# RuihanGao/visual-tactile-synthesis

Hardware: AMD Instinct MI355X
Metric: train_images_per_sec (higher is better)
Workload: dtype f32; 1 GPU; skitG G+D1+D2 train step, 1024x1024 sketch->(RGB,tactile), 4 images/GPU, 64 tactile patches/image, LPIPS/CLIP terms off (no weights offline); global_batch=4, parallelism=dp1, losses_finite=True, hip_graph=True, d2_visualisation_pass=True, train_only=False, full=False

## Files before the change

### visual-tactile-synthesis_amd/csrc/vts_conv_head.hip

```cpp
#include <limits.h>
#include <stdlib.h>

#include "vts_internal.h"

namespace {

struct HeadK {
  const float* x;
  const float *sc, *sh;
  int64_t ns;
  int C, IH, IW, OH, OW, pad, padx;
  const float* w;
  int ws_ci;
  const float* bias;
  float* out;
  int64_t ons;
  float slope;
  const float* ident;
};

constexpr int HK_TY = 32, HK_TX = 32, HK_PR = HK_TY + 3, HK_PC = HK_TX + 3, HK_PCP = 36;
constexpr int HK_MAXC = 512;

template <int CK>
__global__ __launch_bounds__(1024) void conv_head_kernel(const HeadK p) {
  constexpr int BLOCK = 1024, NG = BLOCK / 256, CPG = CK / NG;
  static_assert(CK % NG == 0, "a chunk splits evenly over the thread groups");
  constexpr int NEL = CK * HK_PR * HK_PC;
  constexpr int NLD = (NEL + BLOCK - 1) / BLOCK;
  __shared__ __attribute__((aligned(16))) float tile[CK][HK_PR][HK_PCP];
  __shared__ __attribute__((aligned(16))) float wl[CK][16];
  __shared__ float ssc[HK_MAXC], ssh[HK_MAXC];
  const int tid = threadIdx.x, n = blockIdx.z;
  const int grp = __builtin_amdgcn_readfirstlane(tid >> 8), t256 = tid & 255;
  const int tx4 = t256 & 7, ty = t256 >> 3;
  const int oy0 = blockIdx.y * HK_TY, ox0 = blockIdx.x * HK_TX;
  const int iy0 = oy0 - p.pad, ix0 = ox0 - p.padx;
  for (int c = tid; c < p.C; c += BLOCK) {
    ssc[c] = p.sc ? p.sc[n * p.C + c] : 1.f;
    ssh[c] = p.sh ? p.sh[n * p.C + c] : 0.f;
  }
  int soff[NLD], sdst[NLD];
  const int64_t plane = (int64_t)p.IH * p.IW;
#pragma unroll
  for (int i = 0; i < NLD; ++i) {
    const int e = i * BLOCK + tid;
    const int c = e / (HK_PR * HK_PC), rem = e - c * (HK_PR * HK_PC);
    const int r = rem / HK_PC, col = rem - r * HK_PC;
    const int iy = iy0 + r, ix = ix0 + col;
    const bool in = e < NEL && iy >= 0 && iy < p.IH && ix >= 0 && ix < p.IW;
    soff[i] = in ? iy * p.IW + ix : -1;
    sdst[i] = e < NEL ? (c * HK_PR + r) * HK_PCP + col : -1;
  }
  const float* xb = p.x + n * p.ns;
  float pv[NLD];
  static_assert(BLOCK <= HK_PR * HK_PC, "one boundary per slot");
  auto chan = [&](int i) {
    const int b = (i * BLOCK) / (HK_PR * HK_PC);
    return b + (tid >= (b + 1) * (HK_PR * HK_PC) - i * BLOCK ? 1 : 0);
  };
  auto load_chunk = [&](int c0) {
#pragma unroll
    for (int i = 0; i < NLD; ++i) {
      const int c = c0 + chan(i);
      pv[i] = (soff[i] >= 0 && c < p.C) ? xb[c * plane + soff[i]] : 0.f;
    }
  };
  auto store_chunk = [&](int c0) {
    float* t = &tile[0][0][0];
#pragma unroll
    for (int i = 0; i < NLD; ++i) {
      const int c = c0 + chan(i);
      if (sdst[i] >= 0) {
        const bool ok = soff[i] >= 0 && c < p.C;
        const int cc = min(c, p.C - 1);
        const float u = fmaf(pv[i], ssc[cc], ssh[cc]);
        t[sdst[i]] = ok ? fmaxf(u, 0.f) + p.slope * fminf(u, 0.f) : 0.f;
      }
    }
    if (tid < CK * 16) {
      const int c = c0 + (tid >> 4);
      wl[tid >> 4][tid & 15] = c < p.C ? p.w[(int64_t)c * p.ws_ci + (tid & 15)] : 0.f;
    }
  };
  float acc[4] = {0.f, 0.f, 0.f, 0.f};
  __syncthreads();
  load_chunk(0);
  store_chunk(0);
  __syncthreads();
  for (int c0 = 0; c0 < p.C; c0 += CK) {
    const bool more = c0 + CK < p.C;
    if (more) load_chunk(c0 + CK);
#pragma unroll
    for (int cg = 0; cg < CPG; ++cg) {
      const int c = grp * CPG + cg;
#pragma unroll
      for (int ky = 0; ky < 4; ++ky) {
        const f32x4 a = *reinterpret_cast<const f32x4*>(&tile[c][ty + ky][tx4 * 4]);
        const f32x4 b = *reinterpret_cast<const f32x4*>(&tile[c][ty + ky][tx4 * 4 + 4]);
        const f32x4 wv = *reinterpret_cast<const f32x4*>(&wl[c][ky * 4]);
        const float v[8] = {a[0], a[1], a[2], a[3], b[0], b[1], b[2], b[3]};
#pragma unroll
        for (int kx = 0; kx < 4; ++kx)
#pragma unroll
          for (int j = 0; j < 4; ++j) acc[j] = fmaf(v[j + kx], wv[kx], acc[j]);
      }
    }
    __syncthreads();
    if (more) {
      store_chunk(c0 + CK);
      __syncthreads();
    }
  }
  f32x4* red = reinterpret_cast<f32x4*>(&tile[0][0][0]);
  if (grp > 0) red[(grp - 1) * 256 + t256] = (f32x4){acc[0], acc[1], acc[2], acc[3]};
  __syncthreads();
  if (grp > 0) return;
#pragma unroll
  for (int g = 1; g < NG; ++g) {
    const f32x4 v = red[(g - 1) * 256 + t256];
#pragma unroll
    for (int j = 0; j < 4; ++j) acc[j] += v[j];
  }
  const float bias = p.bias ? p.bias[0] : 0.f;
  const int y = oy0 + ty;
  if (y < p.OH) {
    float* o = p.out + n * p.ons + (int64_t)y * p.OW;
#pragma unroll
    for (int j = 0; j < 4; ++j) {
      const int x = ox0 + tx4 * 4 + j;
      if (x < p.OW) o[x] = acc[j] + bias;
    }
  }
}

struct HeadSK {
  const float* x;
  const float *sc, *sh;
  int64_t ns;
  int C, N, IH, IW, OH, OW, pad, padx;
  const float* w;
  int ws_ci;
  const float* bias;
  float* out;
  int64_t ons;
  float slope;
  int IPB, PH, PW, CK;
};

__global__ __launch_bounds__(256) void conv_head_small_kernel(const HeadSK p) {
  extern __shared__ __attribute__((aligned(16))) float smem[];
  float* tile = smem;
  float* wl = smem + p.IPB * p.CK * p.PH * p.PW;
  const int tid = threadIdx.x;
  const int n0 = blockIdx.x * p.IPB;
  const int nimg = min(p.IPB, p.N - n0);
  const int plane = p.PH * p.PW, ohw = p.OH * p.OW, ihw = p.IH * p.IW;
  const int img = tid / ohw, r = tid - img * ohw;
  const int oy = r / p.OW, ox = r - oy * p.OW;
  const bool active = img < nimg;
  const int base = img * p.CK * plane + oy * p.PW + ox;
  for (int i = tid; i < p.IPB * p.CK * plane; i += 256) tile[i] = 0.f;
  float acc = 0.f;
  for (int c0 = 0; c0 < p.C; c0 += p.CK) {
    __syncthreads();
    const int total = nimg * p.CK * ihw;
    for (int e0 = tid; e0 < total; e0 += 256 * 8) {
      float raw[8], fsc[8], fsh[8];
      int dst[8];
#pragma unroll
      for (int j = 0; j < 8; ++j) {
        const int e = e0 + j * 256;
        const int ee = min(e, total - 1);
        const int ic = ee / ihw, q = ee - ic * ihw;
        const int im = ic / p.CK, c = ic - im * p.CK;
        const int y = q / p.IW, x = q - y * p.IW;
        const int cc = min(c0 + c, p.C - 1), n = n0 + im;
        raw[j] = p.x[n * p.ns + (int64_t)cc * ihw + q];
        fsc[j] = p.sc ? p.sc[n * p.C + cc] : 1.f;
        fsh[j] = p.sh ? p.sh[n * p.C + cc] : 0.f;
        dst[j] = (e < total && c0 + c < p.C) ? (im * p.CK + c) * plane + (y + p.pad) * p.PW + x + p.padx : -1 - ((im * p.CK + c) * plane + (y + p.pad) * p.PW + x + p.padx);
        if (e >= total) dst[j] = INT_MIN;
      }
#pragma unroll
      for (int j = 0; j < 8; ++j) {
        const float t = fmaf(raw[j], fsc[j], fsh[j]);
        if (dst[j] >= 0) tile[dst[j]] = fmaxf(t, 0.f) + p.slope * fminf(t, 0.f);
        else if (dst[j] != INT_MIN) tile[-1 - dst[j]] = 0.f;
      }
    }
    for (int e = tid; e < p.CK * 16; e += 256) wl[e] = (c0 + (e >> 4) < p.C) ? p.w[(int64_t)(c0 + (e >> 4)) * p.ws_ci + (e & 15)] : 0.f;
    __syncthreads();
    if (active) {
#pragma unroll 4
      for (int c = 0; c < p.CK; ++c) {
        const float* t = tile + base + c * plane;
#pragma unroll
        for (int ky = 0; ky < 4; ++ky)
#pragma unroll
          for (int kx = 0; kx < 4; ++kx) acc = fmaf(t[ky * p.PW + kx], wl[c * 16 + ky * 4 + kx], acc);
      }
    }
  }
  if (active) p.out[(n0 + img) * p.ons + r] = acc + (p.bias ? p.bias[0] : 0.f);
}

}

int vts_conv_head_try(const vts_conv_desc* d, hipStream_t st) {
  static const int off = vts_tune_set("VTS_NO_HEAD") ? 1 : 0;
  if (off || d->transposed || d->stride != 1 || d->Cout != 1 || d->in1.data || d->dmask.data || d->accumulate || d->act_out != VTS_ACT_NONE)
    return VTS_ERR_UNSUPPORTED;
  if (d->in0.C > HK_MAXC || d->in0.C < 8 || (int64_t)d->IH * d->IW * d->in0.C >= (1ll << 31)) return VTS_ERR_UNSUPPORTED;
  if ((int64_t)d->OH * d->OW < 1024) {
    const int padx = d->pad + d->pad_dx;
    if (d->N < 32 || d->OH * d->OW > 256 || d->pad < 0 || padx < 0 || d->IH + d->pad < d->OH + 3 - d->pad || d->IW + padx < d->OW + 3 - padx)
      return VTS_ERR_UNSUPPORTED;
    HeadSK q;
    q.x = d->in0.data; q.sc = d->in0.scale; q.sh = d->in0.shift; q.ns = d->in0.nstride; q.C = d->in0.C; q.N = d->N;
    q.IH = d->IH; q.IW = d->IW; q.OH = d->OH; q.OW = d->OW; q.pad = d->pad; q.padx = padx;
    q.w = d->w; q.ws_ci = d->ws_ci; q.bias = d->bias; q.out = d->out; q.ons = d->out_nstride; q.slope = vts_slope(d->act_in);
    q.PH = d->IH + 2 * d->pad; q.PW = d->IW + 2 * padx;
    q.IPB = 256 / (d->OH * d->OW);
    q.CK = d->in0.C;
    auto bytes = [&]() { return (int64_t)(q.IPB * q.CK * q.PH * q.PW + q.CK * 16) * 4; };
    while (q.IPB > 2 && bytes() > 60 * 1024) --q.IPB;
    if (bytes() > 60 * 1024) {
      q.CK = 16;
      q.IPB = 256 / (d->OH * d->OW);
      while (q.IPB > 1 && bytes() > 60 * 1024) --q.IPB;
    }
    const int lds = (int)bytes();
    if (lds > 64 * 1024) return VTS_ERR_UNSUPPORTED;
    hipLaunchKernelGGL(conv_head_small_kernel, dim3(cdiv(d->N, q.IPB)), dim3(256), lds, st, q);
    vts_set_kernel("conv_head_small_kernel");
    VTS_CHECK_LAUNCH("vts_conv4x4 (head, small maps)");
    return VTS_OK;
  }
  HeadK k;
  k.x = d->in0.data; k.sc = d->in0.scale; k.sh = d->in0.shift; k.ns = d->in0.nstride; k.C = d->in0.C;
  k.IH = d->IH; k.IW = d->IW; k.OH = d->OH; k.OW = d->OW; k.pad = d->pad; k.padx = d->pad + d->pad_dx;
  k.w = d->w; k.ws_ci = d->ws_ci; k.bias = d->bias; k.out = d->out; k.ons = d->out_nstride;
  k.slope = vts_slope(d->act_in);
  k.ident = nullptr;
  dim3 grid(cdiv(d->OW, HK_TX), cdiv(d->OH, HK_TY), d->N);
  hipLaunchKernelGGL((conv_head_kernel<8>), grid, dim3(1024), 0, st, k);
  vts_set_kernel("conv_head_kernel<8>");
  VTS_CHECK_LAUNCH("vts_conv4x4 (head)");
  return VTS_OK;
}
```

### visual-tactile-synthesis_amd/csrc/vts_wgrad.hip

```cpp
#include <stdio.h>
#include <stdlib.h>

#include "vts_internal.h"

namespace {

struct Src {
  const float *d0, *d1, *sc0, *sh0, *sc1, *sh1;
  int64_t ns0, ns1;
  int C0, C1, C;
  int act;
  float slope;
  const float* ident;
  int plain;
};

struct WgK {
  Src lo, hi;
  int N, LH, LW, HH, HW, pad, padx;
  int cl_groups, ch_groups;
  int tiles_y, tiles_x, ntiles;
  float* part;
  int ablate;
};
// ... 520 lines not shown
        live[j] = img < nimg;
      }
#pragma unroll
      for (int j = 0; j < 8; ++j) {
        const float t = fmaf(raw[j], fsc[j], fsh[j]);
        if (dst[j] >= 0) lo_t[dst[j]] = live[j] ? fmaxf(t, 0.f) + p.lo_slope * fminf(t, 0.f) : 0.f;
      }
    }
    const int hi_total = nimg * p.CH * hhw;
    for (int e0 = tid; e0 < hi_total; e0 += 256 * 8) {
      float raw[8], fsc[8], fsh[8];
      int dst[8];
#pragma unroll
      for (int j = 0; j < 8; ++j) {
        const int e = min(e0 + j * 256, hi_total - 1);
        int r, c, x;
        const int ic = fdiv(e, hhw, inv_hhw, r);
        const int img = fdiv(ic, p.CH, inv_ch, c);
        const int y = fdiv(r, p.HW, inv_hw, x);
        const int n = n0 + img;
        raw[j] = p.hi[n * p.hins + (int64_t)c * hhw + r];
        fsc[j] = p.hisc ? p.hisc[n * p.CH + c] : 1.f;
        fsh[j] = p.hish ? p.hish[n * p.CH + c] : 0.f;
        dst[j] = e0 + j * 256 < hi_total ? img * imgstride + c * p.PLANE + (y + SW_HALO) * p.PW_ + x + SW_HALO : -1;
      }
#pragma unroll
      for (int j = 0; j < 8; ++j) {
        const float t = fmaf(raw[j], fsc[j], fsh[j]);
        if (dst[j] >= 0) hi_t[dst[j]] = fmaxf(t, 0.f) + p.hi_slope * fminf(t, 0.f);
      }
    }
    __syncthreads();
    const int ngroups = (nimg * lhw + 3) >> 2;
    constexpr int UG = (CLT * CHW >= 16) ? 2 : 4;
    for (int g0 = 0; g0 < ngroups; g0 += UG) {
      float a[UG][CLT], b[UG][CHW];
#pragma unroll
      for (int u = 0; u < UG; ++u) {
        const int pos = min(g0 + u, ngroups - 1) * 4 + kq;
#pragma unroll
        for (int t = 0; t < CLT; ++t) a[u][t] = lo_t[(t * 16 + m16) * p.POSP + pos];
        const int base = postab[pos] + tapoff;
#pragma unroll
        for (int c = 0; c < CHW; ++c) b[u][c] = hi_t[base + min(wave * CHW + c, p.CH - 1) * p.PLANE];
      }
#pragma unroll
      for (int u = 0; u < UG; ++u) {
        if (g0 + u < ngroups) {
#pragma unroll
          for (int t = 0; t < CLT; ++t)
#pragma unroll
            for (int c = 0; c < CHW; ++c) acc[t][c] = __builtin_amdgcn_mfma_f32_16x16x4f32(a[u][t], b[u][c], acc[t][c], 0, 0, 0);
        }
      }
    }
    __syncthreads();
  }
  float* part = p.part + (int64_t)blockIdx.x * p.CL * p.CH * 16;
#pragma unroll
  for (int t = 0; t < CLT; ++t)
#pragma unroll
    for (int c = 0; c < CHW; ++c) {
      const int ch = wave * CHW + c;
#pragma unroll
      for (int r = 0; r < 4; ++r) {
        const int cl = t * 16 + kq * 4 + r;
        if (cl < p.CL && ch < p.CH) part[((int64_t)cl * p.CH + ch) * 16 + m16] = acc[t][c][r];
      }
    }
}

struct HeadWK {
  const float* lo;
  int64_t lons;
  const float *hi, *hisc, *hish;
  int64_t hins;
  int CH, N, LH, LW, HH, HW, pad, padx;
  float hi_slope;
  int tiles_y, tiles_x;
  float* part;
};
constexpr int HWG_TY = 16, HWG_TX = 32, HWG_PR = HWG_TY + 3, HWG_PC = HWG_TX + 3, HWG_PCP = 36, HWG_CK = 16, HWG_PLANE = HWG_PR * HWG_PCP;

__global__ __launch_bounds__(256) void wgrad_head_kernel(const HeadWK p) {
  __shared__ __attribute__((aligned(16))) float patch[HWG_CK * HWG_PLANE];
  __shared__ __attribute__((aligned(16))) float dyt[HWG_TY * HWG_PCP];
  const int tid = threadIdx.x;
  const int tile = blockIdx.x;
  const int n = tile / (p.tiles_y * p.tiles_x), rem = tile - n * (p.tiles_y * p.tiles_x);
  const int ty = rem / p.tiles_x, tx = rem - ty * p.tiles_x;
  const int y0 = ty * HWG_TY, x0 = tx * HWG_TX;
  const int hy0 = y0 - p.pad, hx0 = x0 - p.padx;
  for (int e = tid; e < HWG_TY * HWG_TX; e += 256) {
    const int r = e >> 5, c = e & 31;
    const int y = y0 + r, x = x0 + c;
    dyt[r * HWG_PCP + c] = (y < p.LH && x < p.LW) ? p.lo[n * p.lons + (int64_t)y * p.LW + x] : 0.f;
  }
  const int rg = tid & 3, ky = (tid >> 2) & 3, chl = tid >> 4;
  const int64_t hplane = (int64_t)p.HH * p.HW;
  float* part = p.part + (int64_t)tile * p.CH * 16;
  const int lane = tid & 63;
  const int wv = __builtin_amdgcn_readfirstlane(tid >> 6);
  const int ix = hx0 + lane;
  const bool colok = lane < HWG_PC && ix >= 0 && ix < p.HW;
  const int ixc = min(max(ix, 0), p.HW - 1);
  float raw[HWG_CK / 4][HWG_PR];
  auto load_chunk = [&](int c0) {
#pragma unroll
    for (int cc = 0; cc < HWG_CK / 4; ++cc) {
      const int chc = min(c0 + wv + 4 * cc, p.CH - 1);
      const float* src = p.hi + n * p.hins + chc * hplane + ixc;
#pragma unroll
      for (int r = 0; r < HWG_PR; ++r) raw[cc][r] = src[(int64_t)min(max(hy0 + r, 0), p.HH - 1) * p.HW];
    }
  };
  auto store_chunk = [&](int c0) {
#pragma unroll
    for (int cc = 0; cc < HWG_CK / 4; ++cc) {
      const int c = wv + 4 * cc, ch = c0 + c;
      const bool chok = ch < p.CH;
      const int chc = chok ? ch : p.CH - 1;
      const float sc = p.hisc ? p.hisc[n * p.CH + chc] : 1.f, sh = p.hish ? p.hish[n * p.CH + chc] : 0.f;
      float* dstp = patch + c * HWG_PLANE + min(lane, HWG_PCP - 1);
#pragma unroll
      for (int r = 0; r < HWG_PR; ++r) {
        const int iy = hy0 + r;
        const bool ok = chok && colok && iy >= 0 && iy < p.HH;
        const float t = fmaf(raw[cc][r], sc, sh);
        if (lane < HWG_PCP) dstp[r * HWG_PCP] = ok ? fmaxf(t, 0.f) + p.hi_slope * fminf(t, 0.f) : 0.f;
      }
    }
  };
  load_chunk(0);
  for (int c0 = 0; c0 < p.CH; c0 += HWG_CK) {
    __syncthreads();
    store_chunk(c0);
    if (c0 + HWG_CK < p.CH) load_chunk(c0 + HWG_CK);
    __syncthreads();
    float acc[4] = {0.f, 0.f, 0.f, 0.f};
#pragma unroll
    for (int j = 0; j < HWG_TY / 4; ++j) {
      const int r = rg + 4 * j;
      const f32x4* vp = reinterpret_cast<const f32x4*>(patch + chl * HWG_PLANE + (r + ky) * HWG_PCP);
      const f32x4* dp = reinterpret_cast<const f32x4*>(dyt + r * HWG_PCP);
      float v[HWG_PCP], d[HWG_TX];
#pragma unroll
      for (int i = 0; i < HWG_PCP / 4; ++i) {
        const f32x4 t = vp[i];
        v[4 * i] = t[0]; v[4 * i + 1] = t[1]; v[4 * i + 2] = t[2]; v[4 * i + 3] = t[3];
      }
#pragma unroll
      for (int i = 0; i < HWG_TX / 4; ++i) {
        const f32x4 t = dp[i];
        d[4 * i] = t[0]; d[4 * i + 1] = t[1]; d[4 * i + 2] = t[2]; d[4 * i + 3] = t[3];
      }
#pragma unroll
      for (int x = 0; x < HWG_TX; ++x)
#pragma unroll
        for (int kx = 0; kx < 4; ++kx) acc[kx] = fmaf(d[x], v[x + kx], acc[kx]);
    }
#pragma unroll
    for (int kx = 0; kx < 4; ++kx) {
      const float a = acc[kx] + __shfl_xor(acc[kx], 1);
      acc[kx] = a + __shfl_xor(a, 2);
    }
    if (rg == 0 && c0 + chl < p.CH) *reinterpret_cast<f32x4*>(part + (c0 + chl) * 16 + ky * 4) = (f32x4){acc[0], acc[1], acc[2], acc[3]};
  }
}

__global__ __launch_bounds__(1024) void wgrad_reduce_kernel(const float* __restrict__ part, int64_t n, int pw, float* __restrict__ dw,
                                                            int accumulate) {
  __shared__ float red[16][64];
  const int lane = threadIdx.x & 63, w = threadIdx.x >> 6;
  const int64_t i = (int64_t)blockIdx.x * 64 + lane;
  float s = 0.f;
  if (i < n)
    for (int k = w; k < pw; k += 16) s += part[(int64_t)k * n + i];
  red[w][lane] = s;
  __syncthreads();
  if (w == 0 && i < n) {
    float t = 0.f;
#pragma unroll
    for (int k = 0; k < 16; ++k) t += red[k][lane];
    dw[i] = accumulate ? dw[i] + t : t;
  }
}

constexpr int RB_JOBS = 40;
struct ReduceTable {
  int njobs;
  int blk_start[RB_JOBS + 1];
  unsigned char narrow[RB_JOBS];
  vts_reduce_job job[RB_JOBS];
};

constexpr int RB_ELEMS = 256;
__global__ __launch_bounds__(1024) void wgrad_reduce_batch_kernel(const ReduceTable t) {
  __shared__ f32x4 red[16][64];
  int lo = 0, hi = t.njobs - 1;
  while (lo < hi) {
    const int mid = (lo + hi + 1) >> 1;
    if (t.blk_start[mid] <= (int)blockIdx.x) lo = mid;
    else hi = mid - 1;
  }
  const vts_reduce_job& j = t.job[lo];
  const int lane = threadIdx.x & 63, w = threadIdx.x >> 6;
  if (t.narrow[lo]) {
    const int el = lane & 15, cg = lane >> 4;
    const int64_t nb = (int64_t)(blockIdx.x - t.blk_start[lo]) * 64;
    f32x4 sn = {0.f, 0.f, 0.f, 0.f};
    for (int sg = 0; sg < j.nseg; ++sg) {
      const float* part = j.part[sg];
      const int pw = j.pw[sg];
      const bool vec = nb + 64 <= j.nel && (j.nel & 3) == 0 && (reinterpret_cast<uintptr_t>(part) & 15) == 0;
      f32x4 a[8];
#pragma unroll
      for (int u = 0; u < 8; ++u) a[u] = (f32x4){0.f, 0.f, 0.f, 0.f};
      for (int k = w * 4 + cg; k < pw; k += 512) {
#pragma unroll
        for (int u = 0; u < 8; ++u) {
// ... 268 lines not shown
bool dispatch_ns(const WgK& k, const Plan& pl, hipStream_t st) {
  if (S == 2 && pl.ty > 2) {
#define TALL_CASE(CLT, CHT, TY) \
  if (pl.clt == CLT && pl.cht == CHT && pl.ty == TY) { launch_ns_tall<CLT, CHT, TY>(k, pl, st); return true; }
    TALL_CASE(1, 1, 8) TALL_CASE(2, 1, 8)
#undef TALL_CASE
    return false;
  }
#define NS_CASE(CLT, CHT) \
  if (pl.clt == CLT && pl.cht == CHT) { launch_ns<S, CLT, CHT>(k, pl, st); return true; }
#define NS_ROW(CLT) NS_CASE(CLT, 1) NS_CASE(CLT, 2) NS_CASE(CLT, 3) NS_CASE(CLT, 4) NS_CASE(CLT, 5)
  NS_ROW(1) NS_ROW(2) NS_ROW(3) NS_ROW(4) NS_ROW(5)
#undef NS_ROW
#undef NS_CASE
  return false;
}

}


extern "C" int64_t vts_wgrad4x4_ws_floats(const vts_wgrad_desc* d) {
  if (!d) return 0;
  const int64_t CL = d->lo0.C + (d->lo1.data ? d->lo1.C : 0), CH = d->hi0.C + (d->hi1.data ? d->hi1.C : 0);
  const Plan pl = make_plan(d);
  return (int64_t)pl.pw * CL * CH * 16;
}

extern "C" int vts_wgrad4x4(const vts_wgrad_desc* d, float* ws, void* stream) {
  VTS_CHECK_ARG(d && d->lo0.data && d->hi0.data && d->dw && ws, "vts_wgrad4x4: null pointer");
  VTS_CHECK_ARG(d->stride == 1 || d->stride == 2, "vts_wgrad4x4: stride %d unsupported", d->stride);
  VTS_CHECK_ARG(d->LH <= d->HH + 16 && d->LW <= d->HW + 16 && d->pad >= -8 && d->pad <= 8,
                "vts_wgrad4x4: lo %dx%d / pad %d implausible for hi %dx%d s%d", d->LH, d->LW, d->pad, d->HH, d->HW, d->stride);
  const Plan pl = make_plan(d);
  WgK k;
  fill_src(k.lo, d->lo0, d->lo1, d->act_lo);
  fill_src(k.hi, d->hi0, d->hi1, d->act_hi);
  k.N = d->N; k.LH = d->LH; k.LW = d->LW; k.HH = d->HH; k.HW = d->HW; k.pad = d->pad; k.padx = d->pad + d->pad_dx;
  k.cl_groups = pl.cl_groups; k.ch_groups = pl.ch_groups;
  k.tiles_y = pl.tiles_y; k.tiles_x = pl.tiles_x; k.ntiles = pl.ntiles;
  k.part = ws;
  static const int ablate = vts_tune("VTS_ABLATE", 0);
  k.ablate = ablate;
  hipStream_t st = (hipStream_t)stream;
  const int64_t nel = (int64_t)k.lo.C * k.hi.C * 16;
  if (pl.small) {
    SmallWK q;
    q.lo = d->lo0.data; q.losc = d->lo0.scale; q.losh = d->lo0.shift; q.lons = d->lo0.nstride;
    q.hi = d->hi0.data; q.hisc = d->hi0.scale; q.hish = d->hi0.shift; q.hins = d->hi0.nstride;
    q.CL = k.lo.C; q.CH = k.hi.C; q.N = d->N; q.LH = d->LH; q.LW = d->LW; q.HH = d->HH; q.HW = d->HW; q.S = d->stride; q.pad = d->pad;
    q.padx = d->pad + d->pad_dx;
    q.lo_slope = vts_slope(d->act_lo); q.hi_slope = vts_slope(d->act_hi);
    q.IPB = pl.ipb; q.nblocks = pl.nblocks; q.POS = pl.pos; q.POSP = pl.posp; q.PW_ = pl.pwf; q.PLANE = pl.plane;
    q.part = ws;
    bool ok = false;
#define SW_CASE(CLT, CHW)                                                                                                      \
  if (pl.clt == CLT && pl.cht == CHW) {                                                                                        \
    static bool attr = false;                                                                                                  \
    if (!attr) {                                                                                                               \
      (void)hipFuncSetAttribute((const void*)wgrad_small_kernel<CLT, CHW>, hipFuncAttributeMaxDynamicSharedMemorySize, 160 * 1024); \
      attr = true;                                                                                                             \
    }                                                                                                                          \
    hipLaunchKernelGGL((wgrad_small_kernel<CLT, CHW>), dim3(pl.pw), dim3(256), pl.lds_bytes, st, q);                           \
    vts_set_kernel("wgrad_small_kernel<%d, %d>", CLT, CHW);                                                                    \
    ok = true;                                                                                                                 \
  }
    SW_CASE(1, 2) SW_CASE(1, 4) SW_CASE(1, 8) SW_CASE(1, 16) SW_CASE(2, 2) SW_CASE(2, 4) SW_CASE(2, 8) SW_CASE(2, 16) SW_CASE(4, 2) SW_CASE(4, 4)
    SW_CASE(4, 8)
#undef SW_CASE
    VTS_CHECK_ARG(ok, "vts_wgrad4x4: no small-map instance for clt %d chw %d", pl.clt, pl.cht);
    VTS_CHECK_LAUNCH("vts_wgrad4x4 (small maps)");
    if (d->defer) return VTS_OK;
    hipLaunchKernelGGL(wgrad_reduce_kernel, dim3((unsigned)cdiv64(nel, 64)), dim3(1024), 0, st, ws, nel, pl.pw, d->dw, d->accumulate);
    VTS_CHECK_LAUNCH("vts_wgrad4x4 reduce");
    return VTS_OK;
  }
  if (pl.head) {
    HeadWK q;
    q.lo = d->lo0.data; q.lons = d->lo0.nstride;
    q.hi = d->hi0.data; q.hisc = d->hi0.scale; q.hish = d->hi0.shift; q.hins = d->hi0.nstride;
    q.CH = k.hi.C; q.N = d->N; q.LH = d->LH; q.LW = d->LW; q.HH = d->HH; q.HW = d->HW; q.pad = d->pad; q.padx = d->pad + d->pad_dx;
    q.hi_slope = vts_slope(d->act_hi);
    q.tiles_y = pl.tiles_y; q.tiles_x = pl.tiles_x;
    q.part = ws;
    hipLaunchKernelGGL(wgrad_head_kernel, dim3(pl.ntiles), dim3(256), 0, st, q);
    vts_set_kernel("wgrad_head_kernel");
    VTS_CHECK_LAUNCH("vts_wgrad4x4 (single channel)");
    if (d->defer) return VTS_OK;
    hipLaunchKernelGGL(wgrad_reduce_kernel, dim3((unsigned)cdiv64(nel, 64)), dim3(1024), 0, st, ws, nel, pl.pw, d->dw, d->accumulate);
    VTS_CHECK_LAUNCH("vts_wgrad4x4 reduce");
    return VTS_OK;
  }
  if (pl.ns) {
    const bool ok = d->stride == 2 ? dispatch_ns<2>(k, pl, st) : dispatch_ns<1>(k, pl, st);
    VTS_CHECK_ARG(ok, "vts_wgrad4x4: no N-split instance for clt %d cht %d", pl.clt, pl.cht);
    VTS_CHECK_LAUNCH("vts_wgrad4x4 (N-split)");
    if (d->defer) return VTS_OK;
    hipLaunchKernelGGL(wgrad_reduce_kernel, dim3((unsigned)cdiv64(nel, 64)), dim3(1024), 0, st, ws, nel, pl.pw, d->dw, d->accumulate);
    VTS_CHECK_LAUNCH("vts_wgrad4x4 reduce");
    return VTS_OK;
  }
#define WG_CASE(S, CLT, CHT) \
  if (d->stride == S && pl.clt == CLT && pl.cht == CHT) launch_wg<S, CLT, CHT>(k, pl, st);
  WG_CASE(2, 1, 4) WG_CASE(2, 1, 10) WG_CASE(2, 2, 4) WG_CASE(2, 2, 10) WG_CASE(2, 3, 4) WG_CASE(2, 3, 10) WG_CASE(2, 5, 4)
  WG_CASE(1, 1, 4) WG_CASE(1, 1, 10) WG_CASE(1, 2, 4) WG_CASE(1, 2, 10) WG_CASE(1, 3, 4) WG_CASE(1, 3, 10) WG_CASE(1, 5, 4)
#undef WG_CASE
  VTS_CHECK_LAUNCH("vts_wgrad4x4");
  if (d->defer) return VTS_OK;
  hipLaunchKernelGGL(wgrad_reduce_kernel, dim3((unsigned)cdiv64(nel, 64)), dim3(1024), 0, st, ws, nel, pl.pw, d->dw,
                     d->accumulate);
  VTS_CHECK_LAUNCH("vts_wgrad4x4 reduce");
  return VTS_OK;
}

extern "C" int vts_wgrad_reduce_batch(const vts_reduce_job* jobs, int njobs, void* stream) {
  VTS_CHECK_ARG(jobs && njobs >= 0, "vts_wgrad_reduce_batch: null pointer");
  hipStream_t st = (hipStream_t)stream;
  for (int j0 = 0; j0 < njobs; j0 += RB_JOBS) {
    ReduceTable t;
    t.njobs = njobs - j0 < RB_JOBS ? njobs - j0 : RB_JOBS;
    int blocks = 0;
    for (int j = 0; j < t.njobs; ++j) {
      const vts_reduce_job& q = jobs[j0 + j];
      VTS_CHECK_ARG(q.dw && q.nel > 0 && q.nseg >= 1 && q.nseg <= VTS_REDUCE_MAX_SEG, "vts_wgrad_reduce_batch: bad job %d", j0 + j);
      for (int sg = 0; sg < q.nseg; ++sg) VTS_CHECK_ARG(q.part[sg] && q.pw[sg] >= 1, "vts_wgrad_reduce_batch: bad segment %d of job %d", sg, j0 + j);
      t.job[j] = q;
      t.blk_start[j] = blocks;
      int maxpw = 0;
      for (int sg = 0; sg < q.nseg; ++sg) maxpw = q.pw[sg] > maxpw ? q.pw[sg] : maxpw;
      static const int narrow_min = vts_tune("VTS_REDUCE_NARROW_MIN", 256);
      t.narrow[j] = maxpw > narrow_min ? 1 : 0;
      blocks += (int)cdiv64(q.nel, t.narrow[j] ? 64 : RB_ELEMS);
    }
    t.blk_start[t.njobs] = blocks;
    hipLaunchKernelGGL(wgrad_reduce_batch_kernel, dim3((unsigned)blocks), dim3(1024), 0, st, t);
    VTS_CHECK_LAUNCH("vts_wgrad_reduce_batch");
  }
  return VTS_OK;
}
```

### visual-tactile-synthesis_amd/vts/ops.py

```python
import ctypes as C
import os
from . import tune

import torch

from . import lib as L


class Act:

    __slots__ = ("data", "scale", "shift", "mean", "rstd", "padded")

    def __init__(self, data, scale=None, shift=None, mean=None, rstd=None):
        self.data, self.scale, self.shift, self.mean, self.rstd = data, scale, shift, mean, rstd
        self.padded = None

    @property
    def shape(self):
        return self.data.shape

    def operand(self):
        return L.operand(self.data, self.scale, self.shift)


TIMER = None


DETAIL = None


KNOCKOUT = tuple(k for k in tune.get("VTS_KNOCKOUT", "").split(",") if k)


def _run(label, nbytes, flops, fn, *args):
    global DETAIL
    if KNOCKOUT and label.startswith(KNOCKOUT):
        return
    if TIMER is None:
        L.check(fn(*args), label)
        return
    e0, e1 = torch.cuda.Event(enable_timing=True), torch.cuda.Event(enable_timing=True)
    e0.record()
    rc = fn(*args)
    e1.record()
    L.check(rc, label)
    if label.startswith(("conv4x4", "wgrad4x4", "patch_conv4x4", "patch_wgrad4x4", "norm_", "conv3x3_wide", "wgrad3x3_wide")):
        label = L.load().vts_last_kernel().decode()
    TIMER.append((label, nbytes, flops, e0, e1, DETAIL))
    DETAIL = None


def _numel(op):
    return 0


_ws = {}


def workspace(nfloats, device):
    key = (str(device), WS_LANE)
    t = _ws.get(key)
    if t is None or t.numel() < nfloats:
        if t is not None and frozen_ws():
            _retired.append(t)
        t = torch.empty(max(int(nfloats), 2 * (t.numel() if t is not None else 0), 1 << 20), dtype=torch.float32, device=device)
        _ws[key] = t
    return t


_retired = []

_counters = {}
FUSE_FINALIZE = tune.get("VTS_FUSE_FINALIZE", "0") == "1"


def counters(device):
    if not FUSE_FINALIZE:
        return None
    key = (str(device), WS_LANE)
    t = _counters.get(key)
    if t is None:
        t = _counters[key] = torch.zeros(1 << 16, dtype=torch.int32, device=device)
    return t


_WS_HOLDERS = set()


def freeze_ws(owner):
    _WS_HOLDERS.add(owner)


def release_ws(owner):
    _WS_HOLDERS.discard(owner)


def frozen_ws():
    return bool(_WS_HOLDERS)


WS_LANE = 0


def _op(a):
    if a is None:
        return L.Operand(None, None, None, 0, 0)
    if isinstance(a, Act):
        return a.operand()
    if isinstance(a, L.Operand):
        return a
    return L.operand(a)


BWD_SUMS = tune.get("VTS_BWD_SUMS", "1") != "0"
# ... 1319 lines not shown
```

Baseline: 762.0 images/s.

## Rework single-channel head conv and wgrad kernels for occupancy and register prefetch

The large-map head conv moves from a 1024-thread block with a 32x32 tile to a 256-thread, 8-row tile. Each wave now loads whole input columns into registers, double-buffered, and all weights are staged once in dynamic LDS. The small-map head kernel replaces integer division with magic-number multiplies, loads more elements per batch, and reads weights as vector loads. The head wgrad kernel gains a 512-thread variant that splits channels across two halves when there are fewer tiles than compute units, and it prefetches the per-channel affine terms alongside the data. These changes aim at better occupancy and latency hiding in the discriminator head passes, at the cost of more registers and LDS, and dynamic LDS that scales with channel count.

```diff
diff --git a/visual-tactile-synthesis_amd/csrc/vts_conv_head.hip b/visual-tactile-synthesis_amd/csrc/vts_conv_head.hip
--- a/visual-tactile-synthesis_amd/csrc/vts_conv_head.hip
+++ b/visual-tactile-synthesis_amd/csrc/vts_conv_head.hip
@@ -16,120 +16,134 @@
   float* out;
   int64_t ons;
   float slope;
-  const float* ident;
 };
 
-constexpr int HK_TY = 32, HK_TX = 32, HK_PR = HK_TY + 3, HK_PC = HK_TX + 3, HK_PCP = 36;
+constexpr int HK_TX = 32, HK_PC = HK_TX + 3, HK_PCP = 36, HK_CK = 8;
 constexpr int HK_MAXC = 512;
 
-template <int CK>
-__global__ __launch_bounds__(1024) void conv_head_kernel(const HeadK p) {
-  constexpr int BLOCK = 1024, NG = BLOCK / 256, CPG = CK / NG;
-  static_assert(CK % NG == 0, "a chunk splits evenly over the thread groups");
-  constexpr int NEL = CK * HK_PR * HK_PC;
-  constexpr int NLD = (NEL + BLOCK - 1) / BLOCK;
-  __shared__ __attribute__((aligned(16))) float tile[CK][HK_PR][HK_PCP];
-  __shared__ __attribute__((aligned(16))) float wl[CK][16];
-  __shared__ float ssc[HK_MAXC], ssh[HK_MAXC];
-  const int tid = threadIdx.x, n = blockIdx.z;
-  const int grp = __builtin_amdgcn_readfirstlane(tid >> 8), t256 = tid & 255;
-  const int tx4 = t256 & 7, ty = t256 >> 3;
-  const int oy0 = blockIdx.y * HK_TY, ox0 = blockIdx.x * HK_TX;
+template <int RPT>
+__global__ __launch_bounds__(256) void conv_head_kernel(const HeadK p) {
+  constexpr int TY = 8 * RPT, PR = TY + 3, PLANE = PR * HK_PCP;
+  constexpr int CPW = HK_CK / 4;
+  constexpr int NR = CPW * PR;
+  static_assert(3 * 64 * 4 * RPT <= HK_CK * PLANE, "the partial sums of waves 1 .. 3 fit into the patch memory");
+  __shared__ __attribute__((aligned(16))) float tile[HK_CK * PLANE];
+  extern __shared__ __attribute__((aligned(16))) float wl[];
+  const int tid = threadIdx.x, lane = tid & 63, n = blockIdx.z;
+  const int wv = __builtin_amdgcn_readfirstlane(tid >> 6);
+  const int tx4 = lane & 7, tyr = lane >> 3;
+  const int oy0 = blockIdx.y * TY, ox0 = blockIdx.x * HK_TX;
   const int iy0 = oy0 - p.pad, ix0 = ox0 - p.padx;
-  for (int c = tid; c < p.C; c += BLOCK) {
-    ssc[c] = p.sc ? p.sc[n * p.C + c] : 1.f;
-    ssh[c] = p.sh ? p.sh[n * p.C + c] : 0.f;
-  }
-  int soff[NLD], sdst[NLD];
+  const int ix = ix0 + lane;
+  const bool colok = lane < HK_PC && ix >= 0 && ix < p.IW;
+  const int ixc = min(max(ix, 0), p.IW - 1);
   const int64_t plane = (int64_t)p.IH * p.IW;
-#pragma unroll
-  for (int i = 0; i < NLD; ++i) {
-    const int e = i * BLOCK + tid;
-    const int c = e / (HK_PR * HK_PC), rem = e - c * (HK_PR * HK_PC);
-    const int r = rem / HK_PC, col = rem - r * HK_PC;
-    const int iy = iy0 + r, ix = ix0 + col;
-    const bool in = e < NEL && iy >= 0 && iy < p.IH && ix >= 0 && ix < p.IW;
-    soff[i] = in ? iy * p.IW + ix : -1;
-    sdst[i] = e < NEL ? (c * HK_PR + r) * HK_PCP + col : -1;
-  }
-  const float* xb = p.x + n * p.ns;
-  float pv[NLD];
-  static_assert(BLOCK <= HK_PR * HK_PC, "one boundary per slot");
-  auto chan = [&](int i) {
-    const int b = (i * BLOCK) / (HK_PR * HK_PC);
-    return b + (tid >= (b + 1) * (HK_PR * HK_PC) - i * BLOCK ? 1 : 0);
+  const float* xb = p.x + n * p.ns + ixc;
+  auto load_chunk = [&](float(&raw)[NR], float(&aff)[2 * CPW], int c0) {
+#pragma unroll
+    for (int cc = 0; cc < CPW; ++cc) {
+      const int chc = min(c0 + wv + 4 * cc, p.C - 1);
+      const float* src = xb + chc * plane;
+      aff[2 * cc] = p.sc ? p.sc[n * p.C + chc] : 1.f;
+      aff[2 * cc + 1] = p.sh ? p.sh[n * p.C + chc] : 0.f;
+#pragma unroll
+      for (int r = 0; r < PR; ++r) raw[cc * PR + r] = src[(int64_t)min(max(iy0 + r, 0), p.IH - 1) * p.IW];
+    }
   };
-  auto load_chunk = [&](int c0) {
-#pragma unroll
-    for (int i = 0; i < NLD; ++i) {
-      const int c = c0 + chan(i);
-      pv[i] = (soff[i] >= 0 && c < p.C) ? xb[c * plane + soff[i]] : 0.f;
+  auto store_chunk = [&](const float(&raw)[NR], const float(&aff)[2 * CPW], int c0) {
+#pragma unroll
+    for (int cc = 0; cc < CPW; ++cc) {
+      const int c = wv + 4 * cc, ch = c0 + c;
+      const bool chok = ch < p.C;
+      const float sc = aff[2 * cc], sh = aff[2 * cc + 1];
+      float* dst = tile + c * PLANE + min(lane, HK_PCP - 1);
+#pragma unroll
+      for (int r = 0; r < PR; ++r) {
+        const int iy = iy0 + r;
+        const bool ok = chok && colok && iy >= 0 && iy < p.IH;
+        const float u = fmaf(raw[cc * PR + r], sc, sh);
+        if (lane < HK_PCP) dst[r * HK_PCP] = ok ? fmaxf(u, 0.f) + p.slope * fminf(u, 0.f) : 0.f;
+      }
     }
   };
-  auto store_chunk = [&](int c0) {
-    float* t = &tile[0][0][0];
-#pragma unroll
-    for (int i = 0; i < NLD; ++i) {
-      const int c = c0 + chan(i);
-      if (sdst[i] >= 0) {
-        const bool ok = soff[i] >= 0 && c < p.C;
-        const int cc = min(c, p.C - 1);
-        const float u = fmaf(pv[i], ssc[cc], ssh[cc]);
-        t[sdst[i]] = ok ? fmaxf(u, 0.f) + p.slope * fminf(u, 0.f) : 0.f;
-      }
-    }
-    if (tid < CK * 16) {
-      const int c = c0 + (tid >> 4);
-      wl[tid >> 4][tid & 15] = c < p.C ? p.w[(int64_t)c * p.ws_ci + (tid & 15)] : 0.f;
+  float acc[RPT][4];
+#pragma unroll
+  for (int rr = 0; rr < RPT; ++rr)
+#pragma unroll
+    for (int j = 0; j < 4; ++j) acc[rr][j] = 0.f;
+  auto compute = [&](int c0) {
+#pragma unroll
+    for (int cg = 0; cg < CPW; ++cg) {
+      const int c = wv * CPW + cg;
+      if (c0 + c >= p.C) break;
+      float wk[16];
+#pragma unroll
+      for (int k = 0; k < 4; ++k) {
+        const f32x4 t4 = *reinterpret_cast<const f32x4*>(wl + (c0 + c) * 16 + 4 * k);
+        wk[4 * k] = t4[0]; wk[4 * k + 1] = t4[1]; wk[4 * k + 2] = t4[2]; wk[4 * k + 3] = t4[3];
+      }
+      const float* t = tile + c * PLANE + (tyr * RPT) * HK_PCP + tx4 * 4;
+#pragma unroll
+      for (int q = 0; q < RPT + 3; ++q) {
+        const f32x4 a = *reinterpret_cast<const f32x4*>(t + q * HK_PCP);
+        const f32x4 b = *reinterpret_cast<const f32x4*>(t + q * HK_PCP + 4);
+        const float v[8] = {a[0], a[1], a[2], a[3], b[0], b[1], b[2], b[3]};
+#pragma unroll
+        for (int rr = 0; rr < RPT; ++rr) {
+          const int ky = q - rr;
+          if (ky < 0 || ky > 3) continue;
+#pragma unroll
+          for (int kx = 0; kx < 4; ++kx)
+#pragma unroll
+            for (int j = 0; j < 4; ++j) acc[rr][j] = fmaf(v[j + kx], wk[ky * 4 + kx], acc[rr][j]);
+        }
+      }
     }
   };
-  float acc[4] = {0.f, 0.f, 0.f, 0.f};
+  const int nchunks = (p.C + HK_CK - 1) / HK_CK;
+  float rawA[NR], rawB[NR], affA[2 * CPW], affB[2 * CPW];
+  load_chunk(rawA, affA, 0);
+  if (nchunks > 1) load_chunk(rawB, affB, HK_CK);
+  for (int e = tid; e < p.C * 16; e += 256) wl[e] = p.w[(int64_t)(e >> 4) * p.ws_ci + (e & 15)];
+  for (int k = 0; k < nchunks; k += 2) {
+    __syncthreads();
+    store_chunk(rawA, affA, k * HK_CK);
+    if (k + 2 < nchunks) load_chunk(rawA, affA, (k + 2) * HK_CK);
+    __syncthreads();
+    compute(k * HK_CK);
+    if (k + 1 < nchunks) {
+      __syncthreads();
+      store_chunk(rawB, affB, (k + 1) * HK_CK);
+      if (k + 3 < nchunks) load_chunk(rawB, affB, (k + 3) * HK_CK);
+      __syncthreads();
+      compute((k + 1) * HK_CK);
+    }
+  }
   __syncthreads();
-  load_chunk(0);
-  store_chunk(0);
+  f32x4* red = reinterpret_cast<f32x4*>(tile);
+  if (wv > 0) {
+#pragma unroll
+    for (int rr = 0; rr < RPT; ++rr) red[((wv - 1) * RPT + rr) * 64 + lane] = (f32x4){acc[rr][0], acc[rr][1], acc[rr][2], acc[rr][3]};
+  }
   __syncthreads();
-  for (int c0 = 0; c0 < p.C; c0 += CK) {
-    const bool more = c0 + CK < p.C;
-    if (more) load_chunk(c0 + CK);
-#pragma unroll
-    for (int cg = 0; cg < CPG; ++cg) {
-      const int c = grp * CPG + cg;
-#pragma unroll
-      for (int ky = 0; ky < 4; ++ky) {
-        const f32x4 a = *reinterpret_cast<const f32x4*>(&tile[c][ty + ky][tx4 * 4]);
-        const f32x4 b = *reinterpret_cast<const f32x4*>(&tile[c][ty + ky][tx4 * 4 + 4]);
-        const f32x4 wv = *reinterpret_cast<const f32x4*>(&wl[c][ky * 4]);
-        const float v[8] = {a[0], a[1], a[2], a[3], b[0], b[1], b[2], b[3]};
-#pragma unroll
-        for (int kx = 0; kx < 4; ++kx)
-#pragma unroll
-          for (int j = 0; j < 4; ++j) acc[j] = fmaf(v[j + kx], wv[kx], acc[j]);
-      }
-    }
-    __syncthreads();
-    if (more) {
-      store_chunk(c0 + CK);
-      __syncthreads();
-    }
-  }
-  f32x4* red = reinterpret_cast<f32x4*>(&tile[0][0][0]);
-  if (grp > 0) red[(grp - 1) * 256 + t256] = (f32x4){acc[0], acc[1], acc[2], acc[3]};
-  __syncthreads();
-  if (grp > 0) return;
-#pragma unroll
-  for (int g = 1; g < NG; ++g) {
-    const f32x4 v = red[(g - 1) * 256 + t256];
-#pragma unroll
-    for (int j = 0; j < 4; ++j) acc[j] += v[j];
-  }
+  if (wv > 0) return;
   const float bias = p.bias ? p.bias[0] : 0.f;
-  const int y = oy0 + ty;
-  if (y < p.OH) {
-    float* o = p.out + n * p.ons + (int64_t)y * p.OW;
-#pragma unroll
-    for (int j = 0; j < 4; ++j) {
-      const int x = ox0 + tx4 * 4 + j;
-      if (x < p.OW) o[x] = acc[j] + bias;
+#pragma unroll
+  for (int rr = 0; rr < RPT; ++rr) {
+#pragma unroll
+    for (int g = 1; g < 4; ++g) {
+      const f32x4 v = red[((g - 1) * RPT + rr) * 64 + lane];
+#pragma unroll
+      for (int j = 0; j < 4; ++j) acc[rr][j] += v[j];
+    }
+    const int y = oy0 + tyr * RPT + rr;
+    if (y < p.OH) {
+      float* o = p.out + n * p.ons + (int64_t)y * p.OW;
+#pragma unroll
+      for (int j = 0; j < 4; ++j) {
+        const int x = ox0 + tx4 * 4 + j;
+        if (x < p.OW) o[x] = acc[rr][j] + bias;
+      }
     }
   }
 }
@@ -146,44 +160,50 @@
   int64_t ons;
   float slope;
   int IPB, PH, PW, CK;
+  unsigned m_img, m_ihw, m_iw, m_ohw, m_ow;
 };
+
+inline unsigned hs_magic(int d) { return d == 1 ? 0u : (unsigned)(((1ull << 32) + d - 1) / d); }
+__device__ __forceinline__ int hs_div(int e, unsigned m) { return m ? (int)__umulhi((unsigned)e, m) : e; }
+
+constexpr int HS_SB = 12;
 
 __global__ __launch_bounds__(256) void conv_head_small_kernel(const HeadSK p) {
   extern __shared__ __attribute__((aligned(16))) float smem[];
   float* tile = smem;
-  float* wl = smem + p.IPB * p.CK * p.PH * p.PW;
+  float* wl = smem + ((p.IPB * p.CK * p.PH * p.PW + 3) & ~3);
   const int tid = threadIdx.x;
   const int n0 = blockIdx.x * p.IPB;
   const int nimg = min(p.IPB, p.N - n0);
   const int plane = p.PH * p.PW, ohw = p.OH * p.OW, ihw = p.IH * p.IW;
-  const int img = tid / ohw, r = tid - img * ohw;
-  const int oy = r / p.OW, ox = r - oy * p.OW;
+  const int img = hs_div(tid, p.m_ohw), r = tid - img * ohw;
+  const int oy = hs_div(r, p.m_ow), ox = r - oy * p.OW;
   const bool active = img < nimg;
-  const int base = img * p.CK * plane + oy * p.PW + ox;
+  const int base = active ? img * p.CK * plane + oy * p.PW + ox : 0;
   for (int i = tid; i < p.IPB * p.CK * plane; i += 256) tile[i] = 0.f;
   float acc = 0.f;
   for (int c0 = 0; c0 < p.C; c0 += p.CK) {
     __syncthreads();
-    const int total = nimg * p.CK * ihw;
-    for (int e0 = tid; e0 < total; e0 += 256 * 8) {
-      float raw[8], fsc[8], fsh[8];
-      int dst[8];
-#pragma unroll
-      for (int j = 0; j < 8; ++j) {
+    const int per = p.CK * ihw, total = nimg * per;
+    for (int e0 = tid; e0 < total; e0 += 256 * HS_SB) {
+      float raw[HS_SB], fsc[HS_SB], fsh[HS_SB];
+      int dst[HS_SB];
+#pragma unroll
+      for (int j = 0; j < HS_SB; ++j) {
         const int e = e0 + j * 256;
         const int ee = min(e, total - 1);
-        const int ic = ee / ihw, q = ee - ic * ihw;
-        const int im = ic / p.CK, c = ic - im * p.CK;
-        const int y = q / p.IW, x = q - y * p.IW;
+        const int im = hs_div(ee, p.m_img), ic = ee - im * per;
+        const int c = hs_div(ic, p.m_ihw), q = ic - c * ihw;
+        const int y = hs_div(q, p.m_iw), x = q - y * p.IW;
         const int cc = min(c0 + c, p.C - 1), n = n0 + im;
         raw[j] = p.x[n * p.ns + (int64_t)cc * ihw + q];
         fsc[j] = p.sc ? p.sc[n * p.C + cc] : 1.f;
         fsh[j] = p.sh ? p.sh[n * p.C + cc] : 0.f;
-        dst[j] = (e < total && c0 + c < p.C) ? (im * p.CK + c) * plane + (y + p.pad) * p.PW + x + p.padx : -1 - ((im * p.CK + c) * plane + (y + p.pad) * p.PW + x + p.padx);
-        if (e >= total) dst[j] = INT_MIN;
-      }
-#pragma unroll
-      for (int j = 0; j < 8; ++j) {
+        const int at = (im * p.CK + c) * plane + (y + p.pad) * p.PW + x + p.padx;
+        dst[j] = e >= total ? INT_MIN : (c0 + c < p.C ? at : -1 - at);
+      }
+#pragma unroll
+      for (int j = 0; j < HS_SB; ++j) {
         const float t = fmaf(raw[j], fsc[j], fsh[j]);
         if (dst[j] >= 0) tile[dst[j]] = fmaxf(t, 0.f) + p.slope * fminf(t, 0.f);
         else if (dst[j] != INT_MIN) tile[-1 - dst[j]] = 0.f;
@@ -192,13 +212,16 @@
     for (int e = tid; e < p.CK * 16; e += 256) wl[e] = (c0 + (e >> 4) < p.C) ? p.w[(int64_t)(c0 + (e >> 4)) * p.ws_ci + (e & 15)] : 0.f;
     __syncthreads();
     if (active) {
-#pragma unroll 4
+#pragma unroll 2
       for (int c = 0; c < p.CK; ++c) {
         const float* t = tile + base + c * plane;
-#pragma unroll
-        for (int ky = 0; ky < 4; ++ky)
-#pragma unroll
-          for (int kx = 0; kx < 4; ++kx) acc = fmaf(t[ky * p.PW + kx], wl[c * 16 + ky * 4 + kx], acc);
+        const f32x4* wp = reinterpret_cast<const f32x4*>(wl + c * 16);
+#pragma unroll
+        for (int ky = 0; ky < 4; ++ky) {
+          const f32x4 wk = wp[ky];
+#pragma unroll
+          for (int kx = 0; kx < 4; ++kx) acc = fmaf(t[ky * p.PW + kx], wk[kx], acc);
+        }
       }
     }
   }
@@ -221,17 +244,20 @@
     q.IH = d->IH; q.IW = d->IW; q.OH = d->OH; q.OW = d->OW; q.pad = d->pad; q.padx = padx;
     q.w = d->w; q.ws_ci = d->ws_ci; q.bias = d->bias; q.out = d->out; q.ons = d->out_nstride; q.slope = vts_slope(d->act_in);
     q.PH = d->IH + 2 * d->pad; q.PW = d->IW + 2 * padx;
-    q.IPB = 256 / (d->OH * d->OW);
+    const int ohw = d->OH * d->OW, plane = q.PH * q.PW;
+    q.IPB = 256 / ohw;
     q.CK = d->in0.C;
-    auto bytes = [&]() { return (int64_t)(q.IPB * q.CK * q.PH * q.PW + q.CK * 16) * 4; };
+    auto bytes = [&]() { return (int64_t)(((q.IPB * q.CK * plane + 3) & ~3) + q.CK * 16) * 4; };
     while (q.IPB > 2 && bytes() > 60 * 1024) --q.IPB;
     if (bytes() > 60 * 1024) {
       q.CK = 16;
-      q.IPB = 256 / (d->OH * d->OW);
+      q.IPB = 256 / ohw;
       while (q.IPB > 1 && bytes() > 60 * 1024) --q.IPB;
     }
+    if (bytes() > 64 * 1024) return VTS_ERR_UNSUPPORTED;
+    q.m_img = hs_magic(q.CK * d->IH * d->IW); q.m_ihw = hs_magic(d->IH * d->IW); q.m_iw = hs_magic(d->IW);
+    q.m_ohw = hs_magic(ohw); q.m_ow = hs_magic(d->OW);
     const int lds = (int)bytes();
-    if (lds > 64 * 1024) return VTS_ERR_UNSUPPORTED;
     hipLaunchKernelGGL(conv_head_small_kernel, dim3(cdiv(d->N, q.IPB)), dim3(256), lds, st, q);
     vts_set_kernel("conv_head_small_kernel");
     VTS_CHECK_LAUNCH("vts_conv4x4 (head, small maps)");
@@ -242,10 +268,9 @@
   k.IH = d->IH; k.IW = d->IW; k.OH = d->OH; k.OW = d->OW; k.pad = d->pad; k.padx = d->pad + d->pad_dx;
   k.w = d->w; k.ws_ci = d->ws_ci; k.bias = d->bias; k.out = d->out; k.ons = d->out_nstride;
   k.slope = vts_slope(d->act_in);
-  k.ident = nullptr;
-  dim3 grid(cdiv(d->OW, HK_TX), cdiv(d->OH, HK_TY), d->N);
-  hipLaunchKernelGGL((conv_head_kernel<8>), grid, dim3(1024), 0, st, k);
-  vts_set_kernel("conv_head_kernel<8>");
+  dim3 grid(cdiv(d->OW, HK_TX), cdiv(d->OH, 8), d->N);
+  hipLaunchKernelGGL((conv_head_kernel<1>), grid, dim3(256), d->in0.C * 16 * 4, st, k);
+  vts_set_kernel("conv_head_kernel<1>");
   VTS_CHECK_LAUNCH("vts_conv4x4 (head)");
   return VTS_OK;
 }
diff --git a/visual-tactile-synthesis_amd/csrc/vts_wgrad.hip b/visual-tactile-synthesis_amd/csrc/vts_wgrad.hip
--- a/visual-tactile-synthesis_amd/csrc/vts_wgrad.hip
+++ b/visual-tactile-synthesis_amd/csrc/vts_wgrad.hip
@@ -626,60 +626,69 @@
 };
 constexpr int HWG_TY = 16, HWG_TX = 32, HWG_PR = HWG_TY + 3, HWG_PC = HWG_TX + 3, HWG_PCP = 36, HWG_CK = 16, HWG_PLANE = HWG_PR * HWG_PCP;
 
-__global__ __launch_bounds__(256) void wgrad_head_kernel(const HeadWK p) {
-  __shared__ __attribute__((aligned(16))) float patch[HWG_CK * HWG_PLANE];
-  __shared__ __attribute__((aligned(16))) float dyt[HWG_TY * HWG_PCP];
+template <int NT>
+__global__ __launch_bounds__(NT) void wgrad_head_kernel(const HeadWK p) {
+  constexpr int NH = NT / 256, HWG_CPW = HWG_CK / 4, HWG_NR = HWG_CPW * HWG_PR;
+  __shared__ __attribute__((aligned(16))) float wh_static[NH == 1 ? HWG_TY * HWG_PCP + HWG_CK * HWG_PLANE : 4];
+  extern __shared__ __attribute__((aligned(16))) float wh_dynamic[];
+  float* wh_smem = NH == 1 ? wh_static : wh_dynamic;
+  float* dyt = wh_smem;
   const int tid = threadIdx.x;
+  const int half = __builtin_amdgcn_readfirstlane(tid >> 8), t256 = tid & 255;
+  float* patch = wh_smem + HWG_TY * HWG_PCP + half * (HWG_CK * HWG_PLANE);
   const int tile = blockIdx.x;
   const int n = tile / (p.tiles_y * p.tiles_x), rem = tile - n * (p.tiles_y * p.tiles_x);
   const int ty = rem / p.tiles_x, tx = rem - ty * p.tiles_x;
   const int y0 = ty * HWG_TY, x0 = tx * HWG_TX;
   const int hy0 = y0 - p.pad, hx0 = x0 - p.padx;
-  for (int e = tid; e < HWG_TY * HWG_TX; e += 256) {
+  for (int e = tid; e < HWG_TY * HWG_TX; e += NT) {
     const int r = e >> 5, c = e & 31;
     const int y = y0 + r, x = x0 + c;
     dyt[r * HWG_PCP + c] = (y < p.LH && x < p.LW) ? p.lo[n * p.lons + (int64_t)y * p.LW + x] : 0.f;
   }
-  const int rg = tid & 3, ky = (tid >> 2) & 3, chl = tid >> 4;
+  const int rg = t256 & 3, ky = (t256 >> 2) & 3, chl = t256 >> 4;
   const int64_t hplane = (int64_t)p.HH * p.HW;
   float* part = p.part + (int64_t)tile * p.CH * 16;
   const int lane = tid & 63;
-  const int wv = __builtin_amdgcn_readfirstlane(tid >> 6);
+  const int wv = __builtin_amdgcn_readfirstlane((tid >> 6) & 3);
   const int ix = hx0 + lane;
   const bool colok = lane < HWG_PC && ix >= 0 && ix < p.HW;
   const int ixc = min(max(ix, 0), p.HW - 1);
-  float raw[HWG_CK / 4][HWG_PR];
+  float raw[HWG_NR], aff[2 * HWG_CPW];
   auto load_chunk = [&](int c0) {
 #pragma unroll
-    for (int cc = 0; cc < HWG_CK / 4; ++cc) {
+    for (int cc = 0; cc < HWG_CPW; ++cc) {
       const int chc = min(c0 + wv + 4 * cc, p.CH - 1);
       const float* src = p.hi + n * p.hins + chc * hplane + ixc;
-#pragma unroll
-      for (int r = 0; r < HWG_PR; ++r) raw[cc][r] = src[(int64_t)min(max(hy0 + r, 0), p.HH - 1) * p.HW];
+      aff[2 * cc] = p.hisc ? p.hisc[n * p.CH + chc] : 1.f;
+      aff[2 * cc + 1] = p.hish ? p.hish[n * p.CH + chc] : 0.f;
+#pragma unroll
+      for (int r = 0; r < HWG_PR; ++r) raw[cc * HWG_PR + r] = src[(int64_t)min(max(hy0 + r, 0), p.HH - 1) * p.HW];
     }
   };
   auto store_chunk = [&](int c0) {
 #pragma unroll
-    for (int cc = 0; cc < HWG_CK / 4; ++cc) {
+    for (int cc = 0; cc < HWG_CPW; ++cc) {
       const int c = wv + 4 * cc, ch = c0 + c;
       const bool chok = ch < p.CH;
-      const int chc = chok ? ch : p.CH - 1;
-      const float sc = p.hisc ? p.hisc[n * p.CH + chc] : 1.f, sh = p.hish ? p.hish[n * p.CH + chc] : 0.f;
+      const float sc = aff[2 * cc], sh = aff[2 * cc + 1];
       float* dstp = patch + c * HWG_PLANE + min(lane, HWG_PCP - 1);
 #pragma unroll
       for (int r = 0; r < HWG_PR; ++r) {
         const int iy = hy0 + r;
         const bool ok = chok && colok && iy >= 0 && iy < p.HH;
-        const float t = fmaf(raw[cc][r], sc, sh);
+        const float t = fmaf(raw[cc * HWG_PR + r], sc, sh);
         if (lane < HWG_PCP) dstp[r * HWG_PCP] = ok ? fmaxf(t, 0.f) + p.hi_slope * fminf(t, 0.f) : 0.f;
       }
     }
   };
-  load_chunk(0);
-  for (int c0 = 0; c0 < p.CH; c0 += HWG_CK) {
+  const int cstep = NH * HWG_CK;
+  load_chunk(half * HWG_CK);
+  for (int cb = 0; cb < p.CH; cb += cstep) {
+    const int c0 = cb + half * HWG_CK;
     __syncthreads();
     store_chunk(c0);
-    if (c0 + HWG_CK < p.CH) load_chunk(c0 + HWG_CK);
+    if (cb + cstep < p.CH) load_chunk(c0 + cstep);
     __syncthreads();
     float acc[4] = {0.f, 0.f, 0.f, 0.f};
 #pragma unroll
@@ -1114,7 +1123,30 @@
     q.hi_slope = vts_slope(d->act_hi);
     q.tiles_y = pl.tiles_y; q.tiles_x = pl.tiles_x;
     q.part = ws;
-    hipLaunchKernelGGL(wgrad_head_kernel, dim3(pl.ntiles), dim3(256), 0, st, q);
+    static int cus = 0;
+    if (!cus) {
+      int dev = 0, n = 0;
+      if (hipGetDevice(&dev) != hipSuccess || hipDeviceGetAttribute(&n, hipDeviceAttributeMultiprocessorCount, dev) != hipSuccess || n <= 0) {
+        vts_set_error("vts_wgrad4x4 (single channel): cannot query the compute-unit count");
+        return VTS_ERR_LAUNCH;
+      }
+      cus = n;
+    }
+    if (pl.ntiles < cus) {
+      const int lds = (HWG_TY * HWG_PCP + 2 * HWG_CK * HWG_PLANE) * 4;
+      static bool attr = false;
+      if (!attr) {
+        const hipError_t ea = hipFuncSetAttribute((const void*)wgrad_head_kernel<512>, hipFuncAttributeMaxDynamicSharedMemorySize, lds);
+        if (ea != hipSuccess) {
+          vts_set_error("vts_wgrad4x4 (single channel): hipFuncSetAttribute(max dynamic LDS %d bytes) failed: %s", lds, hipGetErrorString(ea));
+          return VTS_ERR_LAUNCH;
+        }
+        attr = true;
+      }
+      hipLaunchKernelGGL(wgrad_head_kernel<512>, dim3(pl.ntiles), dim3(512), lds, st, q);
+    } else {
+      hipLaunchKernelGGL(wgrad_head_kernel<256>, dim3(pl.ntiles), dim3(256), 0, st, q);
+    }
     vts_set_kernel("wgrad_head_kernel");
     VTS_CHECK_LAUNCH("vts_wgrad4x4 (single channel)");
     if (d->defer) return VTS_OK;
diff --git a/visual-tactile-synthesis_amd/vts/ops.py b/visual-tactile-synthesis_amd/vts/ops.py
--- a/visual-tactile-synthesis_amd/vts/ops.py
+++ b/visual-tactile-synthesis_amd/vts/ops.py
@@ -29,7 +29,11 @@
 DETAIL = None
 
 
-KNOCKOUT = tuple(k for k in tune.get("VTS_KNOCKOUT", "").split(",") if k)
+_KO = tune.get("VTS_KNOCKOUT", "")
+KNOCKOUT = tuple(k for k in _KO.split(";" if ";" in _KO else ",") if k)
+for _k in KNOCKOUT:
+    if _k.count("<") != _k.count(">"):
+        raise ValueError("VTS_KNOCKOUT: %r is a piece of a label that contains commas; separate the labels with ';' (%r)" % (_k, _KO))
 
 
 def _run(label, nbytes, flops, fn, *args):
```

Result: no change. 773.2 images/s (median of 3 runs) (+1.5%).
